# nolan-h-hamilton/ROCCO

Measured on AMD Instinct MI355X. Metric: loci/sec to converged solve, hg38 50bp K=100; BED3 intervals bit-exact, higher is better.
Workload: dtype f64

## Files before the change

### include/rocco_hip.h

```cpp
#ifndef ROCCO_HIP_H
#define ROCCO_HIP_H

#include <stddef.h>
#include <stdint.h>

#ifdef __cplusplus
extern "C" {
#endif

#define ROCCO_HIP_OK 0
#define ROCCO_HIP_ENOMEM (-1)
#define ROCCO_HIP_EINVAL (-2)
#define ROCCO_HIP_EHIP (-3)

#define ROCCO_HIP_PATH_CERTIFIED 1
#define ROCCO_HIP_PATH_EXACT 2
#define ROCCO_HIP_PATH_TRIVIAL 3
#define ROCCO_HIP_PATH_SPINE 4

typedef struct rocco_hip_solver rocco_hip_solver;

int rocco_hip_abi_version(void);

const char *rocco_hip_last_error(void);
// ... 53 lines not shown
    int max_iter;
    uint8_t *solution_dev;
} rocco_hip_budget_task;

typedef struct {
    double selection_penalty;
    double penalized_value;
    long long selected_count;
    int evaluations;
    int path;
    int passes;
    int zone_iters;
    long long n_diff;
    int maps;
} rocco_hip_budget_result;

int rocco_hip_solve_budget_batch_f64(rocco_hip_solver *solver, size_t n_tasks,
                                     const rocco_hip_budget_task *tasks,
                                     rocco_hip_budget_result *results, void *stream);

int rocco_hip_solve_budget_batch_stats_f64(rocco_hip_solver *solver, size_t n_tasks,
                                           const rocco_hip_budget_task *tasks, const double *score_stats_host,
                                           rocco_hip_budget_result *results, void *stream);

typedef struct {
    long long count;
    long long uncertain;
    long long effect;
    long long max_run;
} rocco_hip_probe_stats;

int rocco_hip_delta_probe_f64(rocco_hip_solver *solver, const double *scores_dev,
                              const double *switch_costs_dev, double gamma, size_t n,
                              const uint8_t *emap_dev, const double *lambdas, size_t n_lambdas,
                              rocco_hip_probe_stats *stats_out, void *stream);

int rocco_hip_delta_build_map_f64(rocco_hip_solver *solver, const double *scores_dev,
                                  const double *switch_costs_dev, double gamma, size_t n,
                                  double lambda_ref, double margin, uint8_t *emap_dev, void *stream);

int rocco_hip_delta_build_map_lean_f64(rocco_hip_solver *solver, const double *scores_dev, double gamma, size_t n,
                                       double lambda_ref, double margin, uint8_t *emap_dev, void *stream);

typedef struct {
    long long count_lo, count_hi;
    long long n_diff;
// ... 355 lines not shown
```

### rocco_amd/_native.py

```python
from __future__ import annotations

import contextlib
import ctypes
import os
import threading
from typing import Optional

_HERE = os.path.dirname(os.path.abspath(__file__))
LIB_PATH = os.environ.get("ROCCO_HIP_LIBRARY") or os.path.join(_HERE, "librocco_hip.so")

OK, ENOMEM, EINVAL, EHIP = 0, -1, -2, -3
PATH_CERTIFIED, PATH_EXACT, PATH_TRIVIAL, PATH_SPINE = 1, 2, 3, 4

c_double_p = ctypes.POINTER(ctypes.c_double)
c_ll_p = ctypes.POINTER(ctypes.c_longlong)
c_int_p = ctypes.POINTER(ctypes.c_int)
c_size_p = ctypes.POINTER(ctypes.c_size_t)


class BudgetTask(ctypes.Structure):
    _fields_ = [
        ("scores_dev", ctypes.c_void_p),
        ("switch_costs_dev", ctypes.c_void_p),
        ("gamma", ctypes.c_double),
# ... 70 lines not shown
      ctypes.c_void_p, ctypes.c_void_p]),
    ("rocco_hip_score_mean", ctypes.c_int,
     [ctypes.c_void_p, ctypes.c_void_p, ctypes.c_int, ctypes.c_size_t, ctypes.c_size_t, ctypes.c_size_t,
      ctypes.c_void_p, ctypes.c_void_p]),
    ("rocco_hip_score_mad", ctypes.c_int,
     [ctypes.c_void_p, ctypes.c_void_p, ctypes.c_int, ctypes.c_size_t, ctypes.c_size_t, ctypes.c_size_t,
      ctypes.c_void_p, ctypes.c_void_p]),
    ("rocco_hip_score_percentile_range", ctypes.c_int,
     [ctypes.c_void_p, ctypes.c_void_p, ctypes.c_int, ctypes.c_size_t, ctypes.c_size_t, ctypes.c_size_t, ctypes.c_int,
      ctypes.c_double, ctypes.c_int, ctypes.c_double, ctypes.c_void_p, ctypes.c_void_p]),
    ("rocco_hip_score_std", ctypes.c_int,
     [ctypes.c_void_p, ctypes.c_void_p, ctypes.c_int, ctypes.c_size_t, ctypes.c_size_t, ctypes.c_size_t, ctypes.c_int,
      ctypes.c_void_p, ctypes.c_void_p]),
    ("rocco_hip_score_trimmed_std", ctypes.c_int,
     [ctypes.c_void_p, ctypes.c_void_p, ctypes.c_int, ctypes.c_size_t, ctypes.c_size_t, ctypes.c_size_t, ctypes.c_int, ctypes.c_int,
      ctypes.c_int, ctypes.c_void_p, ctypes.c_void_p]),
    ("rocco_hip_solve_penalized_chain_f64", ctypes.c_int,
     [ctypes.c_void_p, ctypes.c_void_p, ctypes.c_void_p, ctypes.c_double, ctypes.c_size_t,
      ctypes.c_double, ctypes.c_void_p, c_double_p, c_ll_p, c_int_p, ctypes.c_void_p]),
    ("rocco_hip_solve_budget_batch_f64", ctypes.c_int,
     [ctypes.c_void_p, ctypes.c_size_t, ctypes.POINTER(BudgetTask), ctypes.POINTER(BudgetResult),
      ctypes.c_void_p]),
    ("rocco_hip_solve_budget_batch_stats_f64", ctypes.c_int,
     [ctypes.c_void_p, ctypes.c_size_t, ctypes.POINTER(BudgetTask), ctypes.c_void_p, ctypes.POINTER(BudgetResult),
      ctypes.c_void_p]),
    ("rocco_hip_delta_model_lean_f64", ctypes.c_int,
     [ctypes.c_void_p, ctypes.c_void_p, ctypes.c_double, ctypes.c_size_t, ctypes.c_void_p, c_double_p, ctypes.c_size_t,
      c_ll_p, c_ll_p, ctypes.c_void_p]),
    ("rocco_hip_delta_probe_f64", ctypes.c_int,
     [ctypes.c_void_p, ctypes.c_void_p, ctypes.c_void_p, ctypes.c_double, ctypes.c_size_t, ctypes.c_void_p,
      c_double_p, ctypes.c_size_t, ctypes.POINTER(ProbeStats), ctypes.c_void_p]),
    ("rocco_hip_delta_build_map_f64", ctypes.c_int,
     [ctypes.c_void_p, ctypes.c_void_p, ctypes.c_void_p, ctypes.c_double, ctypes.c_size_t,
      ctypes.c_double, ctypes.c_double, ctypes.c_void_p, ctypes.c_void_p]),
    ("rocco_hip_delta_build_map_lean_f64", ctypes.c_int,
     [ctypes.c_void_p, ctypes.c_void_p, ctypes.c_double, ctypes.c_size_t, ctypes.c_double, ctypes.c_double, ctypes.c_void_p,
      ctypes.c_void_p]),
    ("rocco_hip_delta_bound_rounds_f64", ctypes.c_int,
     [ctypes.c_void_p, ctypes.c_void_p, ctypes.c_double, ctypes.c_size_t, c_double_p, c_int_p, ctypes.c_int,
      c_double_p, c_ll_p, c_ll_p, ctypes.c_void_p]),
    ("rocco_hip_delta_spine_f64", ctypes.c_int,
     [ctypes.c_void_p, ctypes.c_void_p, ctypes.c_void_p, ctypes.c_double, ctypes.c_size_t, ctypes.c_void_p,
      c_double_p, ctypes.c_size_t, ctypes.c_int, ctypes.c_void_p, c_ll_p, ctypes.c_void_p]),
    ("rocco_hip_delta_window_f64", ctypes.c_int,
     [ctypes.c_void_p, ctypes.c_void_p, ctypes.c_void_p, ctypes.c_double, ctypes.c_size_t, ctypes.c_void_p,
      ctypes.c_double, ctypes.c_double, ctypes.c_void_p, ctypes.POINTER(WindowStats), ctypes.c_void_p]),
# ... 348 lines not shown
```

### rocco_amd/csrc/api.hip

```cpp
#include <map>
#include <memory>
#include <mutex>
#include "kernels.h"
#include <atomic>

#include "budget.h"
#include "inflate_core.h"
#include "bigwig_sections.h"

#include <algorithm>
#include <cmath>
#include <new>

namespace rocco {

static thread_local std::string g_last_error;

void set_last_error(const std::string &msg) { g_last_error = msg; }

static std::atomic<long long> g_buffer_growths{0};

int DeviceBuffer::reserve(size_t want)
{
    if (want <= bytes) {
// ... 372 lines not shown
    ROCCO_HIP_TRY(hipSetDevice(solver->device)); (void)hipGetLastError();
    return solve_budget_batch(solver, n_tasks, tasks, results, (hipStream_t)stream);
}

int rocco_hip_solve_budget_batch_stats_f64(rocco_hip_solver *solver, size_t n_tasks, const rocco_hip_budget_task *tasks,
                                           const double *score_stats_host, rocco_hip_budget_result *results, void *stream)
{
    if (solver == nullptr || (n_tasks > 0 && (tasks == nullptr || results == nullptr))) {
        return ROCCO_HIP_EINVAL;
    }
    for (size_t t = 0; t < n_tasks; ++t) {
        if (tasks[t].scores_dev == nullptr || tasks[t].n == 0 || tasks[t].n >= ((size_t)1 << 31) ||
            tasks[t].solution_dev == nullptr || tasks[t].max_iter < 0) {
            return ROCCO_HIP_EINVAL;
        }
        if (score_stats_host != nullptr && !(score_stats_host[3 * t] <= score_stats_host[3 * t + 1])) {
            return ROCCO_HIP_EINVAL;
        }
    }
    ROCCO_HIP_TRY(hipSetDevice(solver->device)); (void)hipGetLastError();
    return solve_budget_batch(solver, n_tasks, tasks, results, (hipStream_t)stream, score_stats_host);
}

int rocco_hip_delta_model_lean_f64(rocco_hip_solver *solver, const double *scores_dev, double gamma, size_t n,
                                   const uint8_t *emap_dev, const double *lambdas, size_t n_lambdas, long long *counts_out,
                                   long long *open_out, void *stream)
{
    if (solver == nullptr || scores_dev == nullptr || emap_dev == nullptr || n < 2 || n >= ((size_t)1 << 31) ||
        (n_lambdas > 0 && (lambdas == nullptr || counts_out == nullptr || open_out == nullptr))) {
        return ROCCO_HIP_EINVAL;
    }
    ROCCO_HIP_TRY(hipSetDevice(solver->device)); (void)hipGetLastError();
    return delta_model_lean(solver, scores_dev, gamma, n, emap_dev, lambdas, n_lambdas, counts_out, open_out, (hipStream_t)stream);
}

int rocco_hip_delta_probe_f64(rocco_hip_solver *solver, const double *scores_dev,
                              const double *switch_costs_dev, double gamma, size_t n,
                              const uint8_t *emap_dev, const double *lambdas, size_t n_lambdas,
                              rocco_hip_probe_stats *stats_out, void *stream)
{
    if (solver == nullptr || scores_dev == nullptr || n == 0 || n >= ((size_t)1 << 31) ||
        (n_lambdas > 0 && (lambdas == nullptr || stats_out == nullptr))) {
        return ROCCO_HIP_EINVAL;
    }
    ROCCO_HIP_TRY(hipSetDevice(solver->device)); (void)hipGetLastError();
    return delta_probe(solver, scores_dev, switch_costs_dev, gamma, n, emap_dev, lambdas, n_lambdas,
// ... 1534 lines not shown
```

### rocco_amd/csrc/budget.h

```cpp
#pragma once

#include "kernels.h"

namespace rocco {

int solve_fixed_penalty(rocco_hip_solver *solver, const double *scores_dev,
                        const double *switch_costs_dev, double gamma, size_t n, double lambda,
                        uint8_t *solution_dev, double *value_out, long long *count_out, int *path_out,
                        hipStream_t stream);

int solve_budget_batch(rocco_hip_solver *solver, size_t n_tasks, const rocco_hip_budget_task *tasks,
                       rocco_hip_budget_result *results, hipStream_t stream, const double *score_stats_host = nullptr);

}

namespace rocco {

int delta_probe(rocco_hip_solver *solver, const double *scores_dev, const double *switch_costs_dev,
                double gamma, size_t n, const uint8_t *emap_dev, const double *lambdas, size_t n_lambdas,
                rocco_hip_probe_stats *stats_out, hipStream_t stream);

int delta_spine(rocco_hip_solver *solver, const double *scores_dev, const double *switch_costs_dev,
                double gamma, size_t n, const uint8_t *emap_dev, const double *lambdas, size_t n_lambdas,
                int solution_index, uint8_t *solution_dev, long long *counts_out, hipStream_t stream);

int delta_build_map(rocco_hip_solver *solver, const double *scores_dev, const double *switch_costs_dev,
                    double gamma, size_t n, double lambda_ref, double margin, uint8_t *emap_dev,
                    hipStream_t stream);

int delta_bound_rounds(rocco_hip_solver *solver, const double *scores_dev, double gamma, size_t n,
                       const double *lambdas, const int *round_sizes, int n_rounds, double *lambdas_used_out,
                       long long *counts_out, long long *level_len_out, hipStream_t stream);

int delta_window(rocco_hip_solver *solver, const double *scores_dev, const double *switch_costs_dev,
                 double gamma, size_t n, const uint8_t *emap_dev, double lambda_lo, double lambda_hi,
// ... 13 lines not shown
```

### rocco_amd/csrc/budget.hip

```cpp
#include "budget.h"

#include <algorithm>
#include <atomic>
#include <chrono>
#include <cmath>
#include <cstdio>
#include <cstdlib>
#include <cstring>
#include <thread>

#include "chain.h"
#include "model_chain.h"
#include "chain_fast.h"
#include "lean.h"
#include "lean_tasks.h"
#include "search.h"

namespace rocco {

namespace {

struct DevProblem {
    const double *scores = nullptr;
    const double *costs = nullptr;
// ... 1996 lines not shown
        if ((rc = solver_->host_back.reserve(bytes_out)) != ROCCO_HIP_OK) return rc;
        char *h = (char *)solver_->host_stage.ptr;
        StatsTask *ht = (StatsTask *)h;
        for (size_t b = 0; b < B; ++b) {
            ht[b].scores = probs[b].scores;
            ht[b].switch_costs = probs[b].costs;
            ht[b].n = (long long)probs[b].n;
        }
        std::memcpy(h + bytes_tasks, blockmap.data(), nbt * sizeof(int2));
        char *dv = (char *)solver_->dev_misc.ptr;
        ROCCO_HIP_TRY(hipMemcpyAsync(dv, h, bytes_tasks + bytes_map, hipMemcpyHostToDevice, stream_));
        double *d_part = (double *)(dv + bytes_tasks + bytes_map);
        double *d_out = (double *)(dv + bytes_tasks + bytes_map + bytes_part);
        if ((rc = launch_stats((const StatsTask *)dv, (int)B, (const int2 *)(dv + bytes_tasks), (int)nbt, d_part,
                               d_out, stream_)) != ROCCO_HIP_OK) {
            return rc;
        }
        ROCCO_HIP_TRY(hipMemcpyAsync(solver_->host_back.ptr, d_out, B * 5 * sizeof(double), hipMemcpyDeviceToHost, stream_));
        ROCCO_HIP_TRY(hipStreamSynchronize(stream_));
        std::memcpy(out.data(), solver_->host_back.ptr, B * 5 * sizeof(double));
        return ROCCO_HIP_OK;
    }

    int chain_rounds_run = 0;
    int chain_search(const std::vector<ChainProblem> &problems, const SearchOptions &opt, std::vector<double> &stats_out,
                     std::vector<Presearch> &pre, bool &ran)
    {
        ran = false;
        const double tc0 = now_us();
        const size_t B = probs.size();
        const bool forced = env_set("ROCCO_HIP_CHAIN");
        if (!env_flag("ROCCO_HIP_CHAIN", true) || solver_->lean == 0 || B == 0 || B > (size_t)kChainMaxProblems ||
            !opt.use_bounds || opt.force_exact || !opt.use_compaction) {
            return ROCCO_HIP_OK;
        }
        bool any = false;
        long long tiles0 = 0;
        for (size_t b = 0; b < B; ++b) {
            any = any || lean_eligible(b);
            tiles0 += lean_tiles(probs[b].n);
            if (probs[b].n >= ((size_t)1 << 31)) {
                return ROCCO_HIP_OK;
            }
        }
        if (!any) {
            return ROCCO_HIP_OK;
        }
        if (tiles0 < env_ll("ROCCO_HIP_CHAIN_MIN_TILES", 4096) && !forced) {
            return ROCCO_HIP_OK;
// ... 9 lines not shown
        tune.wgs = std::max(64, env_int("ROCCO_HIP_CHAIN_WGS", 512));
        tune.pilot_wgs = std::max(64, env_int("ROCCO_HIP_CHAIN_PILOT_WGS", 512));
        tune.pilot_tiles = std::max(2, env_int("ROCCO_HIP_CHAIN_PILOT_TILES", 16));
        tune.big_points = env_int("ROCCO_HIP_CHAIN_BIG_POINTS", 2);
        tune.search_gate = opt.search_gate;
        tune.survey_gate = opt.survey_gate;
        tune.interpolate = env_int("ROCCO_HIP_CHAIN_INTERP", 0);
        tune.spread = env_double("ROCCO_HIP_CHAIN_SPREAD", 0.005);
        if (!(tune.spread > 0.0 && tune.spread < 0.5)) {
            tune.spread = 0.005;
        }
        tune.soft_mult = env_double("ROCCO_HIP_CHAIN_SOFT", 0.8);
        {
            std::vector<double> mults = {2.2, 1.2};
            env_list("ROCCO_HIP_CHAIN_LEVELS", mults);
            tune.n_mults = (int)std::min(mults.size(), (size_t)kChainMaxMults);
            for (int k = 0; k < kChainMaxMults; ++k) {
                tune.mults[k] = (k < tune.n_mults) ? mults[(size_t)k] : 0.0;
            }
        }
        const int R = std::max(1, env_int("ROCCO_HIP_CHAIN_ROUNDS", 12));

        std::vector<int2> blockmap;
        for (size_t b = 0; b < B; ++b) {
            const int nb = (int)((probs[b].n + kFastBlockLoci - 1) / kFastBlockLoci);
            for (int k = 0; k < nb; ++k) {
                blockmap.push_back(make_int2((int)b, k));
            }
        }
        const size_t nbt = blockmap.size();
        Layout lay;
        const size_t o_ctl = lay.at(sizeof(LeanRoundCtl));
        const size_t o_in = lay.at(B * sizeof(ChainInput));
        const size_t o_stasks = lay.at(B * sizeof(StatsTask));
        const size_t o_bmap = lay.at(nbt * sizeof(int2));
        lay.end_upload();
        const size_t up_bytes = lay.uploaded;
        const size_t o_probs = lay.at(B * sizeof(ChainProb));
        const size_t o_stats = lay.at(B * 5 * sizeof(double));
        const size_t o_ctl_back = lay.at(sizeof(LeanRoundCtl));
        const size_t down_bytes = lay.bytes() - o_probs;
        const size_t o_hot = lay.at(B * sizeof(ChainHot));
        const size_t o_pilot = lay.at(B * sizeof(ChainPilot));
        const size_t o_evals = lay.at(B * sizeof(ChainEvals));
        const size_t o_tasks = lay.at(B * sizeof(LeanTask));
        const size_t o_points = lay.at(B * kLeanMaxPoints * sizeof(double));
        const size_t o_results = lay.at(B * kLeanMaxPoints * sizeof(LeanResult));
// ... 2 lines not shown
        const bool want_trace = env_set("ROCCO_HIP_CHAIN_TRACE");
        const size_t o_trace = lay.at((size_t)(R + 2) * 8 * sizeof(long long));
        if ((rc = solver_->dev_chain.reserve(lay.bytes() + 256)) != ROCCO_HIP_OK) return rc;
        if ((rc = solver_->host_chain.reserve(std::max(up_bytes, down_bytes) + 256)) != ROCCO_HIP_OK) return rc;
        char *dv = (char *)solver_->dev_chain.ptr;
        char *h = (char *)solver_->host_chain.ptr;
        std::memset(h, 0, o_in);
        ChainInput *hin = (ChainInput *)(h + o_in);
        StatsTask *hst = (StatsTask *)(h + o_stasks);
        for (size_t b = 0; b < B; ++b) {
            const DevProblem &p = probs[b];
            hin[b].scores = p.scores;
            hin[b].n = (long long)p.n;
            hin[b].gamma = p.gamma;
            hin[b].target = std::max(0LL, std::min(problems[b].target_count, (long long)p.n));
            hin[b].pool_begin = lean_[b].pool_begin;
            hin[b].pool_end = lean_[b].pool_end;
            hin[b].allowed = lean_eligible(b) ? 1 : 0;
            hin[b].can_pilot = can_pilot(b) ? 1 : 0;
            hst[b].scores = p.scores;
            hst[b].switch_costs = p.costs;
            hst[b].n = (long long)p.n;
        }
        std::memcpy(h + o_bmap, blockmap.data(), nbt * sizeof(int2));
        ROCCO_HIP_TRY(hipMemcpyAsync(dv, h, up_bytes, hipMemcpyHostToDevice, stream_));
        if ((rc = launch_stats((const StatsTask *)(dv + o_stasks), (int)B, (const int2 *)(dv + o_bmap), (int)nbt, (double *)(dv + o_part),
                               (double *)(dv + o_stats), stream_)) != ROCCO_HIP_OK) {
            return rc;
        }

        const long long rec_cap = 8 * (tiles0 + (long long)tune.wgs) + 64 * (long long)B;
        if ((rc = reserve_round_scratch(rec_cap, false)) != ROCCO_HIP_OK) return rc;

        ChainArgs A;
        A.n_problems = (int)B;
        A.rec_capacity = (int)std::min<long long>(rec_cap, 0x7FFFFFFF);
        A.inputs = (const ChainInput *)(dv + o_in);
        A.probs = (ChainProb *)(dv + o_probs);
        A.hot = (ChainHot *)(dv + o_hot);
        A.pilot = (ChainPilot *)(dv + o_pilot);
        A.evals = (ChainEvals *)(dv + o_evals);
        A.stats = (const double *)(dv + o_stats);
        A.ctl = (LeanRoundCtl *)(dv + o_ctl);
        A.tasks = (LeanTask *)(dv + o_tasks);
        A.points = (double *)(dv + o_points);
        A.results = (LeanResult *)(dv + o_results);
        A.pre = (LeanCompactTask *)(dv + o_pre);
        A.pool = (char *)solver_->dev_lean_pool.ptr;
        A.trace = want_trace ? (long long *)(dv + o_trace) : nullptr;
        A.tune = tune;
// ... 910 lines not shown
    stats_out->n_diff = w.n_diff;
    stats_out->diff_adjacent = w.diff_adjacent ? 1 : 0;
    stats_out->overflow = w.overflow ? 1 : 0;
    stats_out->max_run = w.max_run;
    for (size_t k = 0; k < 16; ++k) {
        if (k < w.diffs.size()) {
            stats_out->diff_locus[k] = w.diffs[k].locus;
            stats_out->diff_margin_lo[k] = w.diffs[k].margin_lo;
            stats_out->diff_margin_hi[k] = w.diffs[k].margin_hi;
            stats_out->diff_run[k] = w.diffs[k].run;
            stats_out->diff_cls_lo[k] = w.diffs[k].cls_lo;
            stats_out->diff_cls_hi[k] = w.diffs[k].cls_hi;
        } else {
            stats_out->diff_locus[k] = -1;
            stats_out->diff_margin_lo[k] = stats_out->diff_margin_hi[k] = 0.0;
            stats_out->diff_run[k] = 0;
            stats_out->diff_cls_lo[k] = stats_out->diff_cls_hi[k] = 0;
        }
    }
    return ROCCO_HIP_OK;
}

int solve_budget_batch(rocco_hip_solver *solver, size_t n_tasks, const rocco_hip_budget_task *tasks,
                       rocco_hip_budget_result *results, hipStream_t stream, const double *score_stats_host)
{
    HipEvaluator ev(solver, stream);
    std::vector<ChainProblem> problems(n_tasks);
    for (size_t t = 0; t < n_tasks; ++t) {
        DevProblem d;
        d.scores = tasks[t].scores_dev;
        d.costs = (tasks[t].n > 1) ? tasks[t].switch_costs_dev : nullptr;
        d.gamma = tasks[t].gamma;
        d.n = tasks[t].n;
        d.solution = tasks[t].solution_dev;
        ev.probs.push_back(d);
        problems[t].n = tasks[t].n;
        problems[t].gamma = tasks[t].gamma;
        problems[t].target_count = tasks[t].target_count;
        problems[t].sum_costs = tasks[t].sum_costs;
        problems[t].max_iter = tasks[t].max_iter;
    }
    int rc;
    SearchOptions opt;
    opt.force_exact = solver->force_exact != 0;
    opt.spec_depth = solver->spec_depth;
    opt.big_round_loci = ev.env_double("ROCCO_HIP_BIG_ROUND", opt.big_round_loci);
    opt.small_round_loci = ev.env_double("ROCCO_HIP_SMALL_ROUND", opt.small_round_loci);
// ... 3 lines not shown
    opt.use_bounds = ev.env_flag("ROCCO_HIP_BOUNDS", opt.use_bounds);
    opt.search_gate = ev.env_double("ROCCO_HIP_SEARCH_GATE", opt.search_gate);
    if (ev.env_set("ROCCO_HIP_SEARCH_POINTS")) opt.search_points = std::max(1, ev.env_int("ROCCO_HIP_SEARCH_POINTS", 0));
    opt.search_interpolate = ev.env_flag("ROCCO_HIP_SEARCH_INTERP", opt.search_interpolate);
    std::vector<CalibrationResult> res;
    const double t_solve0 = HipEvaluator::now_us();
    ev.marks_on_ = ev.env_int("ROCCO_HIP_TIMING", 0) >= 2;
    ev.mark("solve begins");
    opt.use_compaction = ev.env_flag("ROCCO_HIP_COMPACT", opt.use_compaction);
    opt.pilot_rounds = ev.env_int("ROCCO_HIP_PILOT_ROUNDS", opt.pilot_rounds);
    opt.pilot_points = ev.env_int("ROCCO_HIP_PILOT_POINTS", opt.pilot_points);
    opt.align_maps = ev.env_flag("ROCCO_HIP_ALIGN_MAPS", opt.align_maps);
    opt.align_windows = ev.env_flag("ROCCO_HIP_ALIGN_WINDOWS", opt.align_windows);
    ev.env_list("ROCCO_HIP_PILOT_LEVELS", opt.pilot_levels);
    struct LeanOverride {
        rocco_hip_solver *solver;
        int saved;
        ~LeanOverride() { solver->lean = saved; }
    } lean_override{solver, solver->lean};
    if (ev.env_set("ROCCO_HIP_LEAN")) solver->lean = ev.env_flag("ROCCO_HIP_LEAN", true) ? 1 : 0;
    std::vector<double> chain_stats;
    std::vector<Presearch> presearch;
    bool chained = false;
    if (score_stats_host == nullptr) {
        if ((rc = ev.chain_search(problems, opt, chain_stats, presearch, chained)) != ROCCO_HIP_OK) return rc;
    }
    const double tp0 = HipEvaluator::now_us();
    ev.mark("threshold chain parsed");
    if ((rc = prepare(ev, problems, nullptr, score_stats_host, chained ? &chain_stats : nullptr)) != ROCCO_HIP_OK) return rc;
    const double tp1 = HipEvaluator::now_us();
    if ((rc = calibrate_batch(ev, problems, opt, res, chained ? &presearch : nullptr)) != ROCCO_HIP_OK) return rc;
    const double tp2 = HipEvaluator::now_us();
    ev.mark("calibration ends");
    if ((rc = ev.scatter_all()) != ROCCO_HIP_OK) return rc;
    ROCCO_HIP_TRY(hipStreamSynchronize(stream));
    const double t_prepare = tp1 - tp0, t_calibrate = tp2 - tp1, t_scatter = HipEvaluator::now_us() - tp2;
    g_model_chain_counters[0].fetch_add(ev.model_chains, std::memory_order_relaxed);
    g_model_chain_counters[1].fetch_add(ev.model_chain_facts, std::memory_order_relaxed);
    g_model_chain_counters[2].fetch_add(ev.model_chain_hits, std::memory_order_relaxed);
    g_model_chain_counters[3].fetch_add(ev.model_chain_misses, std::memory_order_relaxed);
    g_model_chain_counters[4].fetch_add(ev.model_chain_written, std::memory_order_relaxed);
    g_model_chain_counters[5].fetch_add(ev.model_chain_windows_answered, std::memory_order_relaxed);
    if (ev.env_set("ROCCO_HIP_DEBUG") || ev.env_set("ROCCO_HIP_TIMING")) {
        const double total = HipEvaluator::now_us() - t_solve0;
        std::fprintf(stderr, "[host] solve %.0f us: %d rounds (%d with rounding-model kernels): in the rounds %.0f us = waiting for the device %.0f "
                             "+ reading results %.0f + preparing and submitting %.0f; search logic and the rest %.0f us\n",
                     total, ev.rounds_all, ev.rounds, ev.t_round_, ev.t_wait_, ev.t_consume_,
                     ev.t_round_ - ev.t_wait_ - ev.t_consume_, total - ev.t_round_);
// ... 34 lines not shown
```

### rocco_amd/csrc/chain.h

```cpp
#pragma once

#include "lean.h"

namespace rocco {

constexpr int kChainMaxProblems = 128;
constexpr int kChainMaxLevels = 8;
constexpr int kChainMaxEvals = 384;
constexpr int kChainMaxPilot = 192;
constexpr int kChainMaxMults = 4;
constexpr int kChainKeep = 4;

struct ChainInput {
    const double *scores;
    long long n;
    double gamma;
    long long target;
    unsigned long long pool_begin, pool_end;
    int allowed;
    int can_pilot;
};

struct ChainLevelReport {
    const double *s;
// ... 86 lines not shown
    int n_problems;
    int rec_capacity;
    const ChainInput *inputs;
    ChainProb *probs;
    ChainHot *hot;
    ChainPilot *pilot;
    ChainEvals *evals;
    const double *stats;
    LeanRoundCtl *ctl;
    LeanTask *tasks;
    double *points;
    LeanResult *results;
    LeanCompactTask *pre;
    char *pool;
    long long *trace;
    unsigned long long *follow;
    int follow_words;
    int follow_ctl_word;
    ChainTuning tune;
};

int launch_chain_director(const ChainArgs &A, int round, int last, hipStream_t stream);

}
```

### rocco_amd/csrc/chain.hip

```cpp
#include "chain.h"

#include <cmath>

namespace rocco {

namespace {

constexpr int kDirectorWaves = 16;
constexpr int kDirectorThreads = 64 * kDirectorWaves;

__device__ __forceinline__ double snap_to_grid(double x, int qexp) { return ldexp(rint(ldexp(x, -qexp)), qexp); }

__device__ __forceinline__ int ceil_log2_exact(double x)
{
    const int e = ilogb(x);
    return (x == ldexp(1.0, e)) ? e : e + 1;
}

__device__ __forceinline__ unsigned long long align_up_dev(unsigned long long x, unsigned long long a) { return (x + a - 1) / a * a; }

__device__ __forceinline__ char *pool_alloc(const ChainArgs &A, ChainHot &H, unsigned long long bytes)
{
    const unsigned long long at = align_up_dev(H.pool_at, 256);
    if (at + bytes > H.pool_end) {
// ... 741 lines not shown
        for (int i = threadIdx.x; i < B * kHotWords; i += kDirectorThreads) {
            dst[i] = src[i];
        }
    }
    if (trace) trace[5] = (long long)wall_clock64();
    if (A.follow != nullptr && (last != 0 || A.ctl->all_done != 0)) {
        __syncthreads();
        const unsigned long long *src = reinterpret_cast<const unsigned long long *>(A.probs);
        unsigned long long *dst = A.follow + 32;
        for (int i = threadIdx.x; i < A.follow_words; i += kDirectorThreads) {
            dst[i] = src[i];
        }
        if (threadIdx.x < (int)(sizeof(LeanRoundCtl) / 8)) {
            dst[A.follow_ctl_word + threadIdx.x] = reinterpret_cast<const unsigned long long *>(A.ctl)[threadIdx.x];
        }
        __threadfence_system();
        __syncthreads();
        if (threadIdx.x == 0) {
            __hip_atomic_store(A.follow, 1ull, __ATOMIC_RELEASE, __HIP_MEMORY_SCOPE_SYSTEM);
        }
    }
}

}

int launch_chain_director(const ChainArgs &A, int round, int last, hipStream_t stream)
{
    hipLaunchKernelGGL(chain_director_kernel, dim3(1), dim3(kDirectorThreads), 0, stream, A, round, last);
    ROCCO_HIP_TRY(hipGetLastError());
    return ROCCO_HIP_OK;
}

}
```

### rocco_amd/csrc/median.hip

```cpp
#include "kernels.h"
#include "select_network.h"

#include <limits>

#ifndef ROCCO_MEDIAN_NT
#define ROCCO_MEDIAN_NT 0
#endif

namespace rocco {

namespace {

template <typename T, int KP, bool EXACT>
__device__ __forceinline__ double median_column(const T *__restrict__ m, int K_runtime, long long n, long long stride,
                                                double *__restrict__ out, long long col0, unsigned lane)
{
    const long long j = col0 + lane;
    if (j >= n) {
        return 0.0;
    }
    const int K = EXACT ? KP : K_runtime;
    const int pad = KP - K;
    const int n_lo = pad / 2;
    double v[KP];
// ... 32 lines not shown
                v[k] = bad ? std::numeric_limits<double>::infinity() : v[k];
            }
        }
    }
    select_middle<KP>(v);
    double r;
    if (K & 1) {
        r = v[KP / 2 - 1];
    } else {
        r = (v[KP / 2 - 1] + v[KP / 2]) / 2.0;
    }
    r = has_nan ? __longlong_as_double(0x7FF8000000000000LL) : r;
    out[j] = r;
    return r;
}

template <typename T, int KP, bool EXACT>
__global__ __launch_bounds__(256) void median_kernel(const T *__restrict__ m, int K_runtime, long long n,
                                                     long long stride, double *__restrict__ out)
{
    median_column<T, KP, EXACT>(m, K_runtime, n, stride, out, (long long)xcd_contiguous_block() * 256, threadIdx.x);
}

template <typename T, int KP, bool EXACT>
__global__ __launch_bounds__(256) void median_batch_kernel(MedianBatch batch)
{
    const unsigned logical = xcd_contiguous_block();
    int ti = -1;
#pragma unroll
    for (int i = 0; i < kMedianBatchMax; ++i) {
        ti += (batch.block_begin[i] <= logical) ? 1 : 0;
    }
    const MedianTask &task = batch.tasks[ti];
    const long long col0 = (long long)(logical - task.block_begin) * 256;
    const long long j = col0 + threadIdx.x;
    const double r = median_column<T, KP, EXACT>((const T *)task.matrix, batch.K, task.n, task.stride, task.out, col0, threadIdx.x);
    if (task.partials != nullptr) {
        const bool valid = j < task.n;
        const bool nan = valid && is_nan_bits(r);
        const double inf = std::numeric_limits<double>::infinity();
        double mn = (valid && !nan) ? r : inf, mx = (valid && !nan) ? r : -inf, ab = (valid && !nan) ? fabs(r) : 0.0;
#pragma unroll
        for (int off = 32; off > 0; off >>= 1) {
            mn = fmin(mn, __shfl_xor(mn, off));
            mx = fmax(mx, __shfl_xor(mx, off));
            ab += __shfl_xor(ab, off);
        }
        const bool any_nan = __ballot(nan) != 0ull;
        if ((threadIdx.x & 63) == 0) {
            double *p = task.partials + 3LL * (4LL * (logical - task.block_begin) + (threadIdx.x >> 6));
            p[0] = mn;
            p[1] = mx;
            p[2] = any_nan ? __longlong_as_double(0x7FF8000000000000LL) : ab;
        }
    }
}

constexpr int kStatsSlices = 64;
struct MedianStatsTask {
    const double *partials;
    long long n_partials;
};
struct MedianStatsBatch {
    MedianStatsTask tasks[kMedianBatchMax];
};

__device__ __forceinline__ void stats_block_reduce(double mn, double mx, double ab, bool nan, double *__restrict__ out)
{
    __shared__ double red[4][3];
#pragma unroll
    for (int off = 32; off > 0; off >>= 1) {
        mn = fmin(mn, __shfl_xor(mn, off));
// ... 714 lines not shown
```

### rocco_amd/dp.py

```python
from __future__ import annotations

import ctypes
import functools
import logging
from typing import Dict, Optional, Tuple, Union

import numpy as np

from . import _native

logger = logging.getLogger(__name__)

ArrayLike = Union[np.ndarray, "torch.Tensor", list, tuple]


def _torch():
    import torch

    return torch


def _device_index(device=None) -> int:
    torch = _torch()
    if not torch.cuda.is_available():
# ... 191 lines not shown
    sol_t, value, count, _ = solve_penalized_chain_device(scores_t, switch_costs, selection_penalty)
    return sol_t.cpu().numpy().astype(np.uint8, copy=False), float(value), int(count)


def _sum_costs(n: int, costs_t, gamma: float) -> float:
    if costs_t is None:
        return sum_constant_like_numpy(gamma, n - 1)
    return float(np.sum(costs_t.cpu().numpy()))


def calibrate_selection_penalty_device(scores_t, switch_costs, target_count: int, max_iter: int = 60):
    return calibrate_batch_device([scores_t], [switch_costs], [target_count], max_iter=max_iter)[0]


def _max_iters(max_iter, k: int):
    if np.ndim(max_iter) == 0:
        return [max(0, int(max_iter))] * k
    steps = [max(0, int(m)) for m in max_iter]
    if len(steps) != k:
        raise ValueError("`max_iter` must be an int or hold one int per problem")
    return steps


def calibrate_batch_device(scores_list, switch_costs_list, target_counts, max_iter=60, score_stats=None):
    torch = _torch()
    lib = _native.load()
    k = len(scores_list)
    if k == 0:
        return []
    device = scores_list[0].device
    tasks = (_native.BudgetTask * k)()
    results = (_native.BudgetResult * k)()
    keep = []
    sols = []
    steps = _max_iters(max_iter, k)
    for i, (s_t, costs, target) in enumerate(zip(scores_list, switch_costs_list, target_counts)):
        n = int(s_t.shape[0])
        if n == 0:
            raise ValueError("`scores` cannot be empty")
        costs_t, gamma = _costs_arg(costs, n, device)
        sol_t = torch.empty(n, dtype=torch.uint8, device=device)
        keep.append((s_t, costs_t))
        sols.append(sol_t)
        tasks[i].scores_dev = s_t.data_ptr()
        tasks[i].switch_costs_dev = costs_t.data_ptr() if costs_t is not None else None
        tasks[i].gamma = gamma
        tasks[i].n = n
        tasks[i].target_count = int(target)
        tasks[i].sum_costs = _sum_costs(n, costs_t, gamma)
        tasks[i].max_iter = steps[i]
        tasks[i].solution_dev = sol_t.data_ptr()
    solver = _native.solver_for(device.index)
    if score_stats is not None:
        stats_h = np.ascontiguousarray(score_stats.numpy() if _is_tensor(score_stats) else score_stats, dtype=np.float64)
        if stats_h.shape != (k, 3):
            raise ValueError("`score_stats` must have shape [len(scores_list), 3]")
        _native.check(lib.rocco_hip_solve_budget_batch_stats_f64(solver.handle, k, tasks, stats_h.ctypes.data, results,
                                                                 _stream_ptr(scores_list[0])),
                      "rocco_hip_solve_budget_batch_stats_f64")
    else:
        _native.check(lib.rocco_hip_solve_budget_batch_f64(solver.handle, k, tasks, results,
                                                           _stream_ptr(scores_list[0])),
                      "rocco_hip_solve_budget_batch_f64")
    out = []
    for i in range(k):
        r = results[i]
        out.append((float(r.selection_penalty), sols[i], float(r.penalized_value), int(r.selected_count),
                    {"evaluations": int(r.evaluations), "path": int(r.path), "passes": int(r.passes),
                     "zone_iters": int(r.zone_iters), "n_diff": int(r.n_diff), "maps": int(r.maps)}))
    return out


def calibrate_selection_penalty(scores, switch_costs, target_count: int,
                                max_iter: int = 60) -> Tuple[float, np.ndarray, float, int]:
    _native.load()
    if not _is_tensor(scores) and np.asarray(scores).shape[0] == 0:
        raise ValueError("`scores` cannot be empty")
    scores_t = _to_device_f64(scores)
    penalty, sol_t, value, count, _ = calibrate_selection_penalty_device(
        scores_t, switch_costs, target_count, max_iter=max_iter)
    return float(penalty), sol_t.cpu().numpy().astype(np.uint8, copy=False), float(value), int(count)

# ... 43 lines not shown
```

### rocco_amd/pipeline.py

```python
from __future__ import annotations

import concurrent.futures
import os
import threading
from typing import Dict, List, Optional, Sequence, Tuple

import numpy as np

from . import _native
from . import dp as _dp
from . import rocco as _rocco
from . import shard as _shard

SOLVE_GROUPS = int(os.environ.get("ROCCO_SOLVE_GROUPS", "1"))
SCORE_FIRST = int(os.environ.get("ROCCO_SCORE_FIRST", "0"))
MEDIAN_STATS = bool(int(os.environ.get("ROCCO_MEDIAN_STATS", "0")))
_pool: Optional[concurrent.futures.ThreadPoolExecutor] = None
_group_state: Dict[Tuple[int, int], tuple] = {}
_group_lock = threading.Lock()


def _group_resources(device_index: int, group: int):
    import torch

    key = (int(device_index), int(group))
    if key not in _group_state:
        _group_state[key] = (_native.Solver(int(device_index)), torch.cuda.Stream(device=int(device_index)))
    return _group_state[key]


class ChromWork:

    def __init__(self, name: str, matrix_t, budget: float, gamma: float, step: int = 50, start: int = 0,
                 scoring: str = "median", wls_params: Optional[dict] = None):
        if scoring not in ("median", "wls"):
            raise ValueError("scoring must be 'median' or 'wls'")
        self.name = name
        self.matrix_t = matrix_t
        self.budget = float(budget)
        self.gamma = float(gamma)
        self.step = int(step)
        self.start = int(start)
        self.n = int(matrix_t.shape[1])
        self.scoring = scoring
        self.wls_params = dict(wls_params or {})


def _score_wls(c: ChromWork):
    import torch

    from . import inference as _inference

    s_t, details = _inference.score_loci_wls_device(c.matrix_t.to(torch.float64), **c.wls_params)
    c._effect_mean = details["mean"]
    return s_t


def _solve_group(chroms: Sequence[ChromWork], scores: list, score_stats=None, units: Optional[Sequence[int]] = None) -> list:
    import torch

    if any(s is None for s in scores):
        score_stats = None
    scores = [s if s is not None else _score_wls(c) for c, s in zip(chroms, scores)]
    targets = [int(np.floor(c.n * c.budget)) for c in chroms]
    solved = _dp.calibrate_batch_device(scores, [c.gamma for c in chroms], targets, score_stats=score_stats)
    out = []
    units = list(range(len(chroms))) if units is None else [int(u) for u in units]
    tables, hosts, offsets = [], [], [0]
    for at in range(0, len(chroms), 48):
        part = solved[at:at + 48]
        selected = sum(int(count) for (_p, _s, _v, count, _i) in part)
        part_t, part_off, part_host = _rocco.decode_runs_table_device(
            [sol_t for (_p, sol_t, _v, _c, _i) in part], units=units[at:at + 48], capacity_rows=max(1024, selected // 2 + 64),
            eager_rows=max(4096, selected // 5))
        tables.append(part_t)
        hosts.append(part_host if len(chroms) <= 48 else part_host.copy())
        offsets += [offsets[-1] + o for o in part_off[1:]]
    table_t = tables[0] if len(tables) == 1 else torch.cat(tables, dim=0)
    host_rows = hosts[0] if len(hosts) == 1 else np.concatenate(hosts, axis=0)
    runs = [(table_t[offsets[i]:offsets[i + 1], 1], table_t[offsets[i]:offsets[i + 1], 2]) for i in range(len(chroms))]
    for i, (c, s_t, (penalty, sol_t, value, count, info), (begin_t, end_t)) in enumerate(zip(chroms, scores, solved, runs)):
        out.append({
            "name": c.name, "n": c.n, "selected_count": count, "selection_penalty": penalty,
            "penalized_objective": value, "path": info["path"], "info": info,
            "begin": begin_t, "end": end_t, "solution": sol_t, "step": c.step, "start": c.start,
            "effect_mean": getattr(c, "_effect_mean", None), "scores": s_t,
            "rows": table_t, "rows_host": host_rows, "row_range": (offsets[i], offsets[i + 1]),
        })
# ... 3 lines not shown
def _group_chunks(order: List[int], n_groups: int) -> List[List[int]]:
    k = len(order)
    base, extra = divmod(k, n_groups)
    out, at = [], 0
    for g in range(n_groups):
        size = base + (1 if g < extra else 0)
        out.append(order[at:at + size])
        at += size
    return [c for c in out if c]


def solve_rank(chroms: Sequence[ChromWork], scores_out: Optional[list] = None, groups: Optional[int] = None,
               median_timing: Optional[list] = None, units: Optional[Sequence[int]] = None):
    import torch

    global _pool
    if len(chroms) == 0:
        return []
    device = chroms[0].matrix_t.device
    n_groups = max(1, min(int(groups if groups is not None else SOLVE_GROUPS), len(chroms), _native.max_side_streams()))
    out: List[Optional[dict]] = [None] * len(chroms)
    units = list(range(len(chroms))) if units is None else [int(u) for u in units]

    def score_all(members: Sequence[ChromWork]):
        med = [c for c in members if c.scoring != "wls"]
        if median_timing is not None and med:
            ev0, ev1 = torch.cuda.Event(enable_timing=True), torch.cuda.Event(enable_timing=True)
            ev0.record(torch.cuda.current_stream(device))
        outs, stats_d = [], None
        if med and MEDIAN_STATS:
            outs, stats_d = _rocco.score_central_tendency_chrom_batch_device([c.matrix_t for c in med], with_stats=True)
        elif med:
            outs = _rocco.score_central_tendency_chrom_batch_device([c.matrix_t for c in med])
        got = dict(zip((id(c) for c in med), outs))
        if median_timing is not None and med:
            ev1.record(torch.cuda.current_stream(device))
            nbytes = sum((c.matrix_t.element_size() * int(c.matrix_t.shape[0]) + 8) * c.n for c in med)
            median_timing.append((ev0, ev1, nbytes))
        stats_h = None
        if stats_d is not None and len(med) == len(members):
            stats_h = torch.empty((len(med), 3), dtype=torch.float64, pin_memory=True)
            stats_h.copy_(stats_d, non_blocking=True)
        for c in med:
            c._effect_mean = got[id(c)]
        return [got.get(id(c)) for c in members], stats_h

    if n_groups == 1:
        scores, stats_h = score_all(chroms)
        if stats_h is not None:
            torch.cuda.current_stream(device).synchronize()
        out = _solve_group(chroms, scores, stats_h, units)
    else:
        order = sorted(range(len(chroms)), key=lambda i: -chroms[i].n)
        members = _group_chunks(order, n_groups)
        with torch.cuda.device(device):
            caller_stream = torch.cuda.current_stream(device)

            def work(group: int, idx: List[int], scores: list, scored, stats_h=None, stats_rows=None):
                solver, stream = _group_resources(device.index, group)
                with torch.cuda.device(device), torch.cuda.stream(stream), _native.use_solver(solver):
                    if stats_h is not None:
                        scored.synchronize()
                        if stats_rows is not None:
                            stats_h = stats_h[stats_rows]
                    else:
                        stream.wait_event(scored)
                    res = _solve_group([chroms[i] for i in idx], scores, stats_h, [units[i] for i in idx])
                    stream.synchronize()
                    kept = None if not res or res[0]["rows_host"] is None else res[0]["rows_host"].copy()
                    for r in res:
                        r["rows_host"] = kept
                for r in res:
                    for key in ("begin", "end", "solution", "scores", "effect_mean", "rows"):
                        t = r.get(key)
                        if t is not None and hasattr(t, "record_stream"):
                            t.record_stream(caller_stream)
                return idx, res

            with _group_lock:
                if _pool is None:
                    _pool = concurrent.futures.ThreadPoolExecutor(max_workers=max(1, _native.max_side_streams()),
                                                                  thread_name_prefix="rocco-solve")
                futures = []
                if SCORE_FIRST:
                    every, stats_all = score_all([chroms[i] for i in order])
                    by_index = dict(zip(order, every))
                    row = {i: k for k, i in enumerate(order)}
                    scored = torch.cuda.Event()
                    scored.record(caller_stream)
                    for g, idx in enumerate(members):
                        rows = [row[i] for i in idx] if stats_all is not None else None
                        futures.append(_pool.submit(work, g, idx, [by_index[i] for i in idx], scored, stats_all, rows))
                else:
                    for g, idx in enumerate(members):
                        scores, stats_h = score_all([chroms[i] for i in idx])
                        scored = torch.cuda.Event()
                        scored.record(caller_stream)
                        futures.append(_pool.submit(work, g, idx, scores, scored, stats_h))
                first_error = None
                for f in futures:
                    try:
                        idx, res = f.result()
                        for i, r in zip(idx, res):
                            out[i] = r
                    except BaseException as exc:
                        if first_error is None:
                            first_error = exc
                if first_error is not None:
                    raise first_error
    if scores_out is not None:
        scores_out.extend(r["scores"] for r in out)
    return out


def interval_rows(results: Sequence[dict], host: bool = True):
    import torch

    tables, seen = [], set()
# ... 39 lines not shown
```

Baseline: 5.681 billion.

## Feed median-kernel score stats on device into chain search, use DPP wave reduction

Adds a device-side score-stats entry point so the per-chromosome min/max/abs-sum produced during median scoring can feed the chain search directly. A tiny expand kernel then replaces the separate stats reduction pass over all loci, and no host round-trip is needed. The median kernel's wave reduction also switches from shfl_xor to DPP row operations, with lane 63 writing the partials. The pipeline path is gated by ROCCO_HIP_PREAMBLE, which defaults to 0 in pipeline.py, so only the DPP change runs by default. The DPP lane-mask logic risks reduction correctness errors.

```diff
diff --git a/include/rocco_hip.h b/include/rocco_hip.h
--- a/include/rocco_hip.h
+++ b/include/rocco_hip.h
@@ -99,6 +99,10 @@
 int rocco_hip_solve_budget_batch_stats_f64(rocco_hip_solver *solver, size_t n_tasks,
                                            const rocco_hip_budget_task *tasks, const double *score_stats_host,
                                            rocco_hip_budget_result *results, void *stream);
+
+int rocco_hip_solve_budget_batch_dstats_f64(rocco_hip_solver *solver, size_t n_tasks,
+                                            const rocco_hip_budget_task *tasks, const double *score_stats_dev,
+                                            rocco_hip_budget_result *results, void *stream);
 
 typedef struct {
     long long count;
diff --git a/rocco_amd/_native.py b/rocco_amd/_native.py
--- a/rocco_amd/_native.py
+++ b/rocco_amd/_native.py
@@ -116,6 +116,9 @@
      [ctypes.c_void_p, ctypes.c_size_t, ctypes.POINTER(BudgetTask), ctypes.POINTER(BudgetResult),
       ctypes.c_void_p]),
     ("rocco_hip_solve_budget_batch_stats_f64", ctypes.c_int,
+     [ctypes.c_void_p, ctypes.c_size_t, ctypes.POINTER(BudgetTask), ctypes.c_void_p, ctypes.POINTER(BudgetResult),
+      ctypes.c_void_p]),
+    ("rocco_hip_solve_budget_batch_dstats_f64", ctypes.c_int,
      [ctypes.c_void_p, ctypes.c_size_t, ctypes.POINTER(BudgetTask), ctypes.c_void_p, ctypes.POINTER(BudgetResult),
       ctypes.c_void_p]),
     ("rocco_hip_delta_model_lean_f64", ctypes.c_int,
diff --git a/rocco_amd/csrc/api.hip b/rocco_amd/csrc/api.hip
--- a/rocco_amd/csrc/api.hip
+++ b/rocco_amd/csrc/api.hip
@@ -418,6 +418,22 @@
     return solve_budget_batch(solver, n_tasks, tasks, results, (hipStream_t)stream, score_stats_host);
 }
 
+int rocco_hip_solve_budget_batch_dstats_f64(rocco_hip_solver *solver, size_t n_tasks, const rocco_hip_budget_task *tasks,
+                                            const double *score_stats_dev, rocco_hip_budget_result *results, void *stream)
+{
+    if (solver == nullptr || (n_tasks > 0 && (tasks == nullptr || results == nullptr))) {
+        return ROCCO_HIP_EINVAL;
+    }
+    for (size_t t = 0; t < n_tasks; ++t) {
+        if (tasks[t].scores_dev == nullptr || tasks[t].n == 0 || tasks[t].n >= ((size_t)1 << 31) ||
+            tasks[t].solution_dev == nullptr || tasks[t].max_iter < 0) {
+            return ROCCO_HIP_EINVAL;
+        }
+    }
+    ROCCO_HIP_TRY(hipSetDevice(solver->device)); (void)hipGetLastError();
+    return solve_budget_batch(solver, n_tasks, tasks, results, (hipStream_t)stream, nullptr, score_stats_dev);
+}
+
 int rocco_hip_delta_model_lean_f64(rocco_hip_solver *solver, const double *scores_dev, double gamma, size_t n,
                                    const uint8_t *emap_dev, const double *lambdas, size_t n_lambdas, long long *counts_out,
                                    long long *open_out, void *stream)
diff --git a/rocco_amd/csrc/budget.h b/rocco_amd/csrc/budget.h
--- a/rocco_amd/csrc/budget.h
+++ b/rocco_amd/csrc/budget.h
@@ -10,7 +10,8 @@
                         hipStream_t stream);
 
 int solve_budget_batch(rocco_hip_solver *solver, size_t n_tasks, const rocco_hip_budget_task *tasks,
-                       rocco_hip_budget_result *results, hipStream_t stream, const double *score_stats_host = nullptr);
+                       rocco_hip_budget_result *results, hipStream_t stream, const double *score_stats_host = nullptr,
+                       const double *score_stats_dev = nullptr);
 
 }
 
diff --git a/rocco_amd/csrc/budget.hip b/rocco_amd/csrc/budget.hip
--- a/rocco_amd/csrc/budget.hip
+++ b/rocco_amd/csrc/budget.hip
@@ -2042,9 +2042,24 @@
         return ROCCO_HIP_OK;
     }
 
+    int fetch_stats3(const double *stats3_dev, std::vector<double> &out)
+    {
+        const size_t B = probs.size();
+        out.assign(3 * B, 0.0);
+        if (B == 0) {
+            return ROCCO_HIP_OK;
+        }
+        int rc;
+        if ((rc = solver_->host_back.reserve(align_up(B * 3 * sizeof(double), 256))) != ROCCO_HIP_OK) return rc;
+        ROCCO_HIP_TRY(hipMemcpyAsync(solver_->host_back.ptr, stats3_dev, B * 3 * sizeof(double), hipMemcpyDeviceToHost, stream_));
+        ROCCO_HIP_TRY(hipStreamSynchronize(stream_));
+        std::memcpy(out.data(), solver_->host_back.ptr, B * 3 * sizeof(double));
+        return ROCCO_HIP_OK;
+    }
+
     int chain_rounds_run = 0;
     int chain_search(const std::vector<ChainProblem> &problems, const SearchOptions &opt, std::vector<double> &stats_out,
-                     std::vector<Presearch> &pre, bool &ran)
+                     std::vector<Presearch> &pre, bool &ran, const double *stats3_dev = nullptr)
     {
         ran = false;
         const double tc0 = now_us();
@@ -2100,7 +2115,7 @@
         const int R = std::max(1, env_int("ROCCO_HIP_CHAIN_ROUNDS", 12));
 
         std::vector<int2> blockmap;
-        for (size_t b = 0; b < B; ++b) {
+        for (size_t b = 0; stats3_dev == nullptr && b < B; ++b) {
             const int nb = (int)((probs[b].n + kFastBlockLoci - 1) / kFastBlockLoci);
             for (int k = 0; k < nb; ++k) {
                 blockmap.push_back(make_int2((int)b, k));
@@ -2149,10 +2164,17 @@
             hst[b].switch_costs = p.costs;
             hst[b].n = (long long)p.n;
         }
-        std::memcpy(h + o_bmap, blockmap.data(), nbt * sizeof(int2));
+        if (nbt > 0) {
+            std::memcpy(h + o_bmap, blockmap.data(), nbt * sizeof(int2));
+        }
         ROCCO_HIP_TRY(hipMemcpyAsync(dv, h, up_bytes, hipMemcpyHostToDevice, stream_));
-        if ((rc = launch_stats((const StatsTask *)(dv + o_stasks), (int)B, (const int2 *)(dv + o_bmap), (int)nbt, (double *)(dv + o_part),
-                               (double *)(dv + o_stats), stream_)) != ROCCO_HIP_OK) {
+        if (stats3_dev != nullptr) {
+            rc = launch_chain_stats_expand(stats3_dev, (double *)(dv + o_stats), (int)B, stream_);
+        } else {
+            rc = launch_stats((const StatsTask *)(dv + o_stasks), (int)B, (const int2 *)(dv + o_bmap), (int)nbt, (double *)(dv + o_part),
+                              (double *)(dv + o_stats), stream_);
+        }
+        if (rc != ROCCO_HIP_OK) {
             return rc;
         }
 
@@ -3109,7 +3131,8 @@
 }
 
 int solve_budget_batch(rocco_hip_solver *solver, size_t n_tasks, const rocco_hip_budget_task *tasks,
-                       rocco_hip_budget_result *results, hipStream_t stream, const double *score_stats_host)
+                       rocco_hip_budget_result *results, hipStream_t stream, const double *score_stats_host,
+                       const double *score_stats_dev)
 {
     HipEvaluator ev(solver, stream);
     std::vector<ChainProblem> problems(n_tasks);
@@ -3159,8 +3182,24 @@
     std::vector<double> chain_stats;
     std::vector<Presearch> presearch;
     bool chained = false;
+    if (score_stats_dev != nullptr && score_stats_host == nullptr) {
+        bool usable = ev.env_int("ROCCO_HIP_PREAMBLE", 1) >= 1;
+        for (size_t t = 0; usable && t < n_tasks; ++t) {
+            usable = (ev.probs[t].costs == nullptr);
+        }
+        if (!usable) {
+            score_stats_dev = nullptr;
+        }
+    } else {
+        score_stats_dev = nullptr;
+    }
+    std::vector<double> fetched_stats;
     if (score_stats_host == nullptr) {
-        if ((rc = ev.chain_search(problems, opt, chain_stats, presearch, chained)) != ROCCO_HIP_OK) return rc;
+        if ((rc = ev.chain_search(problems, opt, chain_stats, presearch, chained, score_stats_dev)) != ROCCO_HIP_OK) return rc;
+        if (!chained && score_stats_dev != nullptr) {
+            if ((rc = ev.fetch_stats3(score_stats_dev, fetched_stats)) != ROCCO_HIP_OK) return rc;
+            score_stats_host = fetched_stats.data();
+        }
     }
     const double tp0 = HipEvaluator::now_us();
     ev.mark("threshold chain parsed");
diff --git a/rocco_amd/csrc/chain.h b/rocco_amd/csrc/chain.h
--- a/rocco_amd/csrc/chain.h
+++ b/rocco_amd/csrc/chain.h
@@ -132,4 +132,6 @@
 
 int launch_chain_director(const ChainArgs &A, int round, int last, hipStream_t stream);
 
+int launch_chain_stats_expand(const double *stats3_dev, double *stats5_dev, int n_problems, hipStream_t stream);
+
 }
diff --git a/rocco_amd/csrc/chain.hip b/rocco_amd/csrc/chain.hip
--- a/rocco_amd/csrc/chain.hip
+++ b/rocco_amd/csrc/chain.hip
@@ -787,6 +787,18 @@
     }
 }
 
+__global__ __launch_bounds__(64) void chain_stats_expand_kernel(const double *__restrict__ stats3, double *__restrict__ stats5,
+                                                                int n_problems)
+{
+    for (int b = threadIdx.x; b < n_problems; b += 64) {
+        stats5[5 * b + 0] = stats3[3 * b + 0];
+        stats5[5 * b + 1] = stats3[3 * b + 1];
+        stats5[5 * b + 2] = 0.0;
+        stats5[5 * b + 3] = 0.0;
+        stats5[5 * b + 4] = stats3[3 * b + 2];
+    }
+}
+
 }
 
 int launch_chain_director(const ChainArgs &A, int round, int last, hipStream_t stream)
@@ -796,4 +808,11 @@
     return ROCCO_HIP_OK;
 }
 
-}
+int launch_chain_stats_expand(const double *stats3_dev, double *stats5_dev, int n_problems, hipStream_t stream)
+{
+    hipLaunchKernelGGL(chain_stats_expand_kernel, dim3(1), dim3(64), 0, stream, stats3_dev, stats5_dev, n_problems);
+    ROCCO_HIP_TRY(hipGetLastError());
+    return ROCCO_HIP_OK;
+}
+
+}
diff --git a/rocco_amd/csrc/median.hip b/rocco_amd/csrc/median.hip
--- a/rocco_amd/csrc/median.hip
+++ b/rocco_amd/csrc/median.hip
@@ -78,6 +78,31 @@
     median_column<T, KP, EXACT>(m, K_runtime, n, stride, out, (long long)xcd_contiguous_block() * 256, threadIdx.x);
 }
 
+template <int CTRL, int ROW_MASK>
+__device__ __forceinline__ double dpp_take(double x, double idle)
+{
+    const long long xb = __double_as_longlong(x), ib = __double_as_longlong(idle);
+    const int lo = __builtin_amdgcn_update_dpp((int)(ib & 0xFFFFFFFFLL), (int)(xb & 0xFFFFFFFFLL), CTRL, ROW_MASK, 0xF, false);
+    const int hi = __builtin_amdgcn_update_dpp((int)(ib >> 32), (int)(xb >> 32), CTRL, ROW_MASK, 0xF, false);
+    return __longlong_as_double(((long long)hi << 32) | (unsigned int)lo);
+}
+
+__device__ __forceinline__ void wave_stats_dpp(double &mn, double &mx, double &ab)
+{
+    const double inf = std::numeric_limits<double>::infinity();
+#define ROCCO_STATS_STEP(CTRL, ROWS)                         \
+    mn = fmin(mn, dpp_take<CTRL, ROWS>(mn, inf));            \
+    mx = fmax(mx, dpp_take<CTRL, ROWS>(mx, -inf));           \
+    ab += dpp_take<CTRL, ROWS>(ab, 0.0);
+    ROCCO_STATS_STEP(0x111, 0xF)
+    ROCCO_STATS_STEP(0x112, 0xF)
+    ROCCO_STATS_STEP(0x114, 0xF)
+    ROCCO_STATS_STEP(0x118, 0xF)
+    ROCCO_STATS_STEP(0x142, 0xA)
+    ROCCO_STATS_STEP(0x143, 0xC)
+#undef ROCCO_STATS_STEP
+}
+
 template <typename T, int KP, bool EXACT>
 __global__ __launch_bounds__(256) void median_batch_kernel(MedianBatch batch)
 {
@@ -96,14 +121,9 @@
         const bool nan = valid && is_nan_bits(r);
         const double inf = std::numeric_limits<double>::infinity();
         double mn = (valid && !nan) ? r : inf, mx = (valid && !nan) ? r : -inf, ab = (valid && !nan) ? fabs(r) : 0.0;
-#pragma unroll
-        for (int off = 32; off > 0; off >>= 1) {
-            mn = fmin(mn, __shfl_xor(mn, off));
-            mx = fmax(mx, __shfl_xor(mx, off));
-            ab += __shfl_xor(ab, off);
-        }
+        wave_stats_dpp(mn, mx, ab);
         const bool any_nan = __ballot(nan) != 0ull;
-        if ((threadIdx.x & 63) == 0) {
+        if ((threadIdx.x & 63) == 63) {
             double *p = task.partials + 3LL * (4LL * (logical - task.block_begin) + (threadIdx.x >> 6));
             p[0] = mn;
             p[1] = mx;
diff --git a/rocco_amd/dp.py b/rocco_amd/dp.py
--- a/rocco_amd/dp.py
+++ b/rocco_amd/dp.py
@@ -237,7 +237,8 @@
     return steps
 
 
-def calibrate_batch_device(scores_list, switch_costs_list, target_counts, max_iter=60, score_stats=None):
+def calibrate_batch_device(scores_list, switch_costs_list, target_counts, max_iter=60, score_stats=None,
+                           score_stats_device=None):
     torch = _torch()
     lib = _native.load()
     k = len(scores_list)
@@ -273,6 +274,13 @@
         _native.check(lib.rocco_hip_solve_budget_batch_stats_f64(solver.handle, k, tasks, stats_h.ctypes.data, results,
                                                                  _stream_ptr(scores_list[0])),
                       "rocco_hip_solve_budget_batch_stats_f64")
+    elif score_stats_device is not None:
+        if (tuple(score_stats_device.shape) != (k, 3) or score_stats_device.dtype != torch.float64
+                or not score_stats_device.is_contiguous() or score_stats_device.device != device):
+            raise ValueError("`score_stats_device` must be a contiguous float64 [len(scores_list), 3] tensor on the scores' device")
+        _native.check(lib.rocco_hip_solve_budget_batch_dstats_f64(solver.handle, k, tasks, score_stats_device.data_ptr(), results,
+                                                                  _stream_ptr(scores_list[0])),
+                      "rocco_hip_solve_budget_batch_dstats_f64")
     else:
         _native.check(lib.rocco_hip_solve_budget_batch_f64(solver.handle, k, tasks, results,
                                                            _stream_ptr(scores_list[0])),
diff --git a/rocco_amd/pipeline.py b/rocco_amd/pipeline.py
--- a/rocco_amd/pipeline.py
+++ b/rocco_amd/pipeline.py
@@ -15,6 +15,12 @@
 SOLVE_GROUPS = int(os.environ.get("ROCCO_SOLVE_GROUPS", "1"))
 SCORE_FIRST = int(os.environ.get("ROCCO_SCORE_FIRST", "0"))
 MEDIAN_STATS = bool(int(os.environ.get("ROCCO_MEDIAN_STATS", "0")))
+
+
+def _preamble() -> int:
+    return int(os.environ.get("ROCCO_HIP_PREAMBLE", "0"))
+
+
 _pool: Optional[concurrent.futures.ThreadPoolExecutor] = None
 _group_state: Dict[Tuple[int, int], tuple] = {}
 _group_lock = threading.Lock()
@@ -56,14 +62,16 @@
     return s_t
 
 
-def _solve_group(chroms: Sequence[ChromWork], scores: list, score_stats=None, units: Optional[Sequence[int]] = None) -> list:
+def _solve_group(chroms: Sequence[ChromWork], scores: list, score_stats=None, units: Optional[Sequence[int]] = None,
+                 score_stats_device=None) -> list:
     import torch
 
     if any(s is None for s in scores):
-        score_stats = None
+        score_stats = score_stats_device = None
     scores = [s if s is not None else _score_wls(c) for c, s in zip(chroms, scores)]
     targets = [int(np.floor(c.n * c.budget)) for c in chroms]
-    solved = _dp.calibrate_batch_device(scores, [c.gamma for c in chroms], targets, score_stats=score_stats)
+    solved = _dp.calibrate_batch_device(scores, [c.gamma for c in chroms], targets, score_stats=score_stats,
+                                        score_stats_device=score_stats_device if score_stats is None else None)
     out = []
     units = list(range(len(chroms))) if units is None else [int(u) for u in units]
     tables, hosts, offsets = [], [], [0]
@@ -113,13 +121,13 @@
     out: List[Optional[dict]] = [None] * len(chroms)
     units = list(range(len(chroms))) if units is None else [int(u) for u in units]
 
-    def score_all(members: Sequence[ChromWork]):
+    def score_all(members: Sequence[ChromWork], device_stats: bool = False):
         med = [c for c in members if c.scoring != "wls"]
         if median_timing is not None and med:
             ev0, ev1 = torch.cuda.Event(enable_timing=True), torch.cuda.Event(enable_timing=True)
             ev0.record(torch.cuda.current_stream(device))
         outs, stats_d = [], None
-        if med and MEDIAN_STATS:
+        if med and (MEDIAN_STATS or device_stats):
             outs, stats_d = _rocco.score_central_tendency_chrom_batch_device([c.matrix_t for c in med], with_stats=True)
         elif med:
             outs = _rocco.score_central_tendency_chrom_batch_device([c.matrix_t for c in med])
@@ -129,18 +137,21 @@
             nbytes = sum((c.matrix_t.element_size() * int(c.matrix_t.shape[0]) + 8) * c.n for c in med)
             median_timing.append((ev0, ev1, nbytes))
         stats_h = None
-        if stats_d is not None and len(med) == len(members):
+        if device_stats:
+            stats_d = stats_d if len(med) == len(members) else None
+        elif stats_d is not None and len(med) == len(members):
             stats_h = torch.empty((len(med), 3), dtype=torch.float64, pin_memory=True)
             stats_h.copy_(stats_d, non_blocking=True)
         for c in med:
             c._effect_mean = got[id(c)]
-        return [got.get(id(c)) for c in members], stats_h
+        return [got.get(id(c)) for c in members], stats_h, (stats_d if device_stats else None)
 
     if n_groups == 1:
-        scores, stats_h = score_all(chroms)
+        device_stats = _preamble() >= 1 and all(c.scoring != "wls" for c in chroms)
+        scores, stats_h, stats_d = score_all(chroms, device_stats)
         if stats_h is not None:
             torch.cuda.current_stream(device).synchronize()
-        out = _solve_group(chroms, scores, stats_h, units)
+        out = _solve_group(chroms, scores, stats_h, units, stats_d)
     else:
         order = sorted(range(len(chroms)), key=lambda i: -chroms[i].n)
         members = _group_chunks(order, n_groups)
@@ -174,7 +185,7 @@
                                                                   thread_name_prefix="rocco-solve")
                 futures = []
                 if SCORE_FIRST:
-                    every, stats_all = score_all([chroms[i] for i in order])
+                    every, stats_all, _ = score_all([chroms[i] for i in order])
                     by_index = dict(zip(order, every))
                     row = {i: k for k, i in enumerate(order)}
                     scored = torch.cuda.Event()
@@ -184,7 +195,7 @@
                         futures.append(_pool.submit(work, g, idx, [by_index[i] for i in idx], scored, stats_all, rows))
                 else:
                     for g, idx in enumerate(members):
-                        scores, stats_h = score_all([chroms[i] for i in idx])
+                        scores, stats_h, _ = score_all([chroms[i] for i in idx])
                         scored = torch.cuda.Event()
                         scored.record(caller_stream)
                         futures.append(_pool.submit(work, g, idx, scores, scored, stats_h))
```

Measured after the change: 5.697 billion, median of 2. No clear change (+0.3%).
